# arun-sub/genomicsbench

Hardware: AMD Instinct MI355X
Metric: bsw_large_gcups (higher is better)
Workload: dtype int32

## Files before the change

genomicsbench_amd/csrc/bsw_kernels.hip:

```cpp
#include "gbx_internal.h"
#include <atomic>
#include <climits>
#include <cstdlib>

namespace gbx {
namespace {

constexpr int NEG = -(1 << 29);
constexpr int BIGJ = 1 << 20;

constexpr int NCLS = 21;
constexpr int CLS_LDS = NCLS - 1;
constexpr int NTB = 32;
constexpr int NBIN = NCLS * NTB;
constexpr int HDR = 1024;
constexpr int REG_SCORE_LIMIT = 1 << 20;

struct BswDev {
    int o_del, e_del, o_ins, e_ins, oe_del, oe_ins, zdrop, end_bonus, w, max_mat;
    uint32_t colword[5];
    int32_t col4[5];
    uint32_t row0[5];
    uint32_t row1[5];
    uint8_t remap[24];
    uint32_t lrow[5];
    int lane_on;
};

struct BswPairs {
    const uint8_t *ref, *qer;
    const int64_t *idr, *idq;
    const int32_t *len1, *len2, *h0;
    gbx_bsw_result *out;
    int packed = 0;
};

constexpr int WS_HDR = 4 * HDR;
struct BswWork {
    int32_t *counts, *cursors, *base, *bad, *order, *wband;
    int32_t *lbase, *lrank, *lorder, *lchunk;
};

__host__ __device__ inline int cls_of(int qlen, int bound)
{
    if (qlen > 1024 || bound >= REG_SCORE_LIMIT) return CLS_LDS;
    if (qlen > 256) return 19;
    if (qlen <= 128) return (qlen - 1) >> 3;
    return qlen <= 160 ? 16 : qlen <= 192 ? 17 : 18;
}
constexpr int LANE_QMAX = 159;
constexpr int LANE_ROWS = 2 * (LANE_QMAX + 1);
constexpr int LANE_BINS = LANE_ROWS * 256;
constexpr int LANE_SCORE_LIMIT = 8192;
constexpr int LANE_COMPACT_LIMIT = 256;
constexpr int LANE_NRANGE = 5;
constexpr int LANE_RANGE_HI[2][LANE_NRANGE] = {{47, 79, 99, 135, LANE_QMAX}, {39, 79, 103, 127, LANE_QMAX}};
__host__ __device__ inline bool lane_ok(int lane_on, int qlen, int tlen, int h0, int max_mat)
{
    return lane_on && qlen >= 1 && qlen <= LANE_QMAX && tlen >= 1 && h0 >= 0 && h0 + qlen * (max_mat > 0 ? max_mat : 0) < LANE_SCORE_LIMIT;
}
__host__ __device__ inline int lane_key(int qlen, int h0, int max_mat)
{
    const int wide = h0 + qlen * (max_mat > 0 ? max_mat : 0) < LANE_COMPACT_LIMIT ? 0 : 1;
    return ((wide * (LANE_QMAX + 1) + qlen) << 8) | (h0 < 255 ? h0 : 255);
}

__host__ __device__ inline int bin_of(int cls, int tlen)
{
    const int tb = tlen >> 4;
    return cls * NTB + (NTB - 1 - (tb < NTB - 1 ? tb : NTB - 1));
}

__device__ inline int imax3(int a, int b, int c) { return max(max(a, b), c); }

template <int CTRL, int ROWMASK = 0xf, int BANKMASK = 0xf>
__device__ inline int dpp(int old, int x)
{
    return __builtin_amdgcn_update_dpp(old, x, CTRL, ROWMASK, BANKMASK, false);
}

template <int CTRL, int ROWMASK = 0xf>
__device__ inline int dppz(int x)
{
    return __builtin_amdgcn_mov_dpp(x, CTRL, ROWMASK, 0xf, true);
}

template <int LPP>
__device__ inline int group_scan_max(int x)
{
    if (LPP == 2) return max(x, dppz<0xa0>(x));
    if (LPP <= 8) {
        x = max(x, dppz<0x90>(x));
        x = max(x, dppz<0x40>(x));
        if (LPP == 8) {
            const int tot = dppz<0xff>(x);
            x = max(x, dpp<0x114, 0xf, 0xa>(0, tot));
        }
        return x;
    }
    x = max(x, dppz<0x111>(x));
    x = max(x, dppz<0x112>(x));
    x = max(x, dppz<0x114>(x));
    x = max(x, dppz<0x118>(x));
    if (LPP >= 32) x = max(x, dpp<0x142, 0xa>(NEG, x));
    if (LPP >= 64) x = max(x, dpp<0x143, 0xc>(NEG, x));
    return x;
}

template <int LPP>
__device__ inline int group_shift_up(int x, int fill, int gl)
{
    if (LPP == 16) return dpp<0x111>(fill, x);
    if (LPP < 16) { const int y = dpp<0x111>(fill, x); return gl == 0 ? fill : y; }
    int y = dpp<0x138>(fill, x);
    return gl == 0 ? fill : y;
}

template <int LPP>
__device__ inline int group_allmax(int x)
{
    if (LPP == 2) return max(x, dppz<0xb1>(x));
    if (LPP <= 8) {
        x = max(x, dppz<0xb1>(x));
        x = max(x, dppz<0x4e>(x));
        if (LPP == 8) x = max(x, dppz<0x141>(x));
        return x;
    }
    if (LPP == 16) {
        x = max(x, dppz<0x121>(x));
        x = max(x, dppz<0x122>(x));
        x = max(x, dppz<0x124>(x));
        x = max(x, dppz<0x128>(x));
        return x;
    }
    x = max(x, dpp<0x111>(x, x));
    x = max(x, dpp<0x112>(x, x));
    x = max(x, dpp<0x114>(x, x));
    x = max(x, dpp<0x118>(x, x));
    x = max(x, dpp<0x142, 0xa>(x, x));
    x = max(x, dpp<0x143, 0xc>(x, x));
    return __builtin_amdgcn_readlane(x, 63);
}

__device__ inline int band_width(const BswDev &prm, int qlen)
{
    const int n_ins = qlen * prm.max_mat + prm.end_bonus - prm.o_ins;
    const int n_del = qlen * prm.max_mat + prm.end_bonus - prm.o_del;
    const int l_ins = n_ins >= 0 ? n_ins / prm.e_ins + 1 : 1;
    const int l_del = n_del >= 0 ? n_del / prm.e_del + 1 : 1;
    return min(prm.w, min(l_ins, l_del));
}

constexpr int CLS_THREADS = 1024;
__global__ void __launch_bounds__(CLS_THREADS) bsw_classify_kernel(BswDev prm, BswPairs P, int64_t n, BswWork W, int pass)
{
    __shared__ int lcount[NBIN];
    __shared__ int lbase[NBIN];
    const int tid = threadIdx.x;
    for (int b = tid; b < NBIN; b += CLS_THREADS) lcount[b] = 0;
    __syncthreads();
    const int64_t k = (int64_t)blockIdx.x * CLS_THREADS + tid;
    int bin = -1, slot = 0;
    if (k < n) {
        const int qlen = P.len2[k], tlen = P.len1[k], h0 = P.h0[k];
        if (qlen < 0 || tlen < 0 || qlen > GBX_BSW_MAX_QLEN || tlen > GBX_BSW_MAX_TLEN) {
            if (pass == 0) {
                gbx_bsw_result r = {-1, -1, -1, -1, -1, -1};
                P.out[k] = r;
                atomicAdd(W.bad, 1);
            }
        } else if (tlen == 0 || qlen == 0) {
            if (pass == 0) {
                gbx_bsw_result r;
                r.score = h0; r.tle = 0; r.qle = 0; r.max_off = 0;
                if (tlen == 0) { r.gtle = 0; r.gscore = -1; }
                else { int left = max(h0 - (prm.o_del + prm.e_del), 0); r.gtle = 1; r.gscore = max(-1, left); }
                P.out[k] = r;
            }
        } else if (lane_ok(prm.lane_on, qlen, tlen, h0, prm.max_mat)) {
        } else {
            const int bound = max(h0, 0) + qlen * max(prm.max_mat, 0);
            bin = bin_of(prm.remap[cls_of(qlen, bound)], tlen);
            slot = atomicAdd(&lcount[bin], 1);
        }
    }
    __syncthreads();
    if (pass == 0) {
        for (int b = tid; b < NBIN; b += CLS_THREADS)
            if (lcount[b]) atomicAdd(&W.counts[b], lcount[b]);
        return;
    }
    for (int b = tid; b < NBIN; b += CLS_THREADS)
        lbase[b] = lcount[b] ? W.base[b] + atomicAdd(&W.cursors[b], lcount[b]) : 0;
    __syncthreads();
    if (bin >= 0) {
        W.order[lbase[bin] + slot] = (int)k;
        W.wband[lbase[bin] + slot] = band_width(prm, P.len2[k]);
    }
}

__global__ void __launch_bounds__(HDR) bsw_scan_kernel(BswWork W)
{
    __shared__ int tmp[HDR];
    const int tid = threadIdx.x;
    const int v = tid < NBIN ? W.counts[tid] : 0;
    tmp[tid] = v;
    __syncthreads();
    for (int d = 1; d < HDR; d <<= 1) {
        const int add = tid >= d ? tmp[tid - d] : 0;
        __syncthreads();
        tmp[tid] += add;
        __syncthreads();
    }
    if (tid <= NBIN) W.base[tid] = tmp[tid] - v;
}

constexpr int rows_min_waves(int cpl) { return cpl >= 17 ? 3 : cpl >= 12 ? 4 : cpl >= 9 ? 5 : cpl >= 7 ? 6 : cpl >= 5 ? 7 : 1; }

template <int LPP, int CPL, bool SYM>
__global__ void __launch_bounds__(256, rows_min_waves(CPL)) bsw_rows_kernel(BswDev prm, BswPairs P, BswWork W, int cls)
{
    constexpr int KB = 10;
    constexpr int GROUPS_PER_BLOCK = 256 / LPP;
    constexpr int NQ = (CPL + 3) / 4;
    static_assert(LPP * CPL <= (1 << KB), "column index must fit the key");
    static_assert(CPL <= 32, "in-lane column index uses 5 bits");

    __shared__ uint2 s_row[8];
    const int tid = threadIdx.x;
    if (tid < 8) s_row[tid] = make_uint2(prm.row0[min(tid, 4)], prm.row1[min(tid, 4)]);
    __syncthreads();

    const int gl = tid & (LPP - 1);
    const int j0 = gl * CPL;
    const int ngroups = gridDim.x * GROUPS_PER_BLOCK;
    int next = blockIdx.x * GROUPS_PER_BLOCK + tid / LPP;

    const bool direct = cls < 0;
    const int first = direct ? 0 : W.base[cls * NTB];
    const int cnt = direct ? -cls : W.base[(cls + 1) * NTB] - first;
    const int32_t *order = W.order + first;
    const int32_t *wband = W.wband + first;

    const int e_ins = prm.e_ins, e_del = prm.e_del, oe_ins = prm.oe_ins, oe_del = prm.oe_del;
    const int lane_tilt = gl * (CPL * e_ins);

    int Hs[CPL + 1], Ev[CPL];
    uint32_t Qp[NQ];
#pragma unroll
    for (int c = 0; c < CPL; ++c) { Hs[c] = 0; Ev[c] = 0; }
#pragma unroll
    for (int c = 0; c < NQ; ++c) Qp[c] = 0;

    int qlen = 1, tlen = 1, w = 0, beg = 0, end = 0, i = 0, pair = 0, lq = 0;
    int best = 0, best_i = -1, best_j = -1, g_i = -1, g_score = -1, off = 0;
    int leftv = 0;
    const uint8_t *tptr = P.ref;
    uint2 rcur = s_row[0];
    int tnext = 0;
    bool active = false, done = false;

    for (;;) {
        if (done) {
            if (gl == lq) {
                gbx_bsw_result r;
                r.score = best; r.tle = best_i + 1; r.gtle = g_i + 1; r.qle = best_j + 1;
                r.gscore = g_score; r.max_off = off;
                P.out[pair] = r;
            }
            done = false; active = false;
            tptr = P.ref; tlen = 1; i = 0;
        }
        if (!active && next < cnt) {
            pair = direct ? next : order[next];
            w = direct ? band_width(prm, P.len2[pair]) : wband[next];
            next += ngroups;
            qlen = P.len2[pair]; tlen = P.len1[pair];
            const int h0 = P.h0[pair];
            const uint8_t *q = P.qer + P.idq[pair];
            tptr = P.ref + P.idr[pair];
#pragma unroll
            for (int c = 0; c < NQ; ++c) Qp[c] = 0;
#pragma unroll
            for (int c = 0; c < CPL; ++c) {
                const int j = j0 + c;
                int qc = j < qlen ? q[j] : 0;
                qc = min(qc, 4);
                Qp[c >> 2] |= (uint32_t)qc << ((c & 3) * 8);
                Hs[c] = j == 0 ? h0 : max(h0 - oe_ins - (j - 1) * e_ins, 0);
                Ev[c] = 0;
            }
            lq = (qlen - 1) / CPL;
            leftv = h0 - prm.o_del - e_del;
            best = h0; best_i = -1; best_j = -1; g_i = -1; g_score = -1; off = 0;
            beg = 0; end = qlen; i = 0;
            rcur = s_row[min((int)tptr[0], 4)];
            tnext = tptr[min(1, tlen - 1)];
            active = true;
        }
        if (!__any(active)) break;

        const int b = max(beg, i - w);
        const int e = min(min(end, i + w + 1), qlen);
        const int left0 = b == 0 ? max(leftv, 0) : 0;
        leftv -= e_del;
        const int lo = b - j0, hi = e - j0;
        uint32_t sw[NQ];
#pragma unroll
        for (int k = 0; k < NQ; ++k) sw[k] = __builtin_amdgcn_perm(rcur.y, rcur.x, Qp[k]);
        rcur = s_row[min(tnext, 4)];
        tnext = tptr[min(i + 2, tlen - 1)];

        int G[CPL];
        int lf = NEG;
#pragma unroll
        for (int c = 0; c < CPL; ++c) {
            const bool p = (c >= lo) & (c < hi);
            const int hsv = Hs[c];
            const int sc = (int)(int8_t)(sw[c >> 2] >> ((c & 3) * 8));
            const int m = (p & (hsv != 0)) ? hsv + sc : 0;
            const int ein = p ? Ev[c] : 0;
            G[c] = imax3(m, ein, lf);
            const int mo = m - oe_ins;
            lf = imax3(lf - e_ins, mo, 0);
            Ev[c] = imax3(ein - e_del, SYM ? mo : m - oe_del, 0);
        }
        const int carry = group_scan_max<LPP>(lf + lane_tilt) - lane_tilt;
        int X = group_shift_up<LPP>(carry, NEG, gl);

        int kl = 0, hl = 0;
#pragma unroll
        for (int c = 0; c < CPL; ++c) {
            int h = max(G[c], X);
            X -= e_ins;
            const bool pr = c < hi;
            Hs[c + 1] = pr ? h : Hs[c + 1];
            hl = pr ? h : hl;
            h = pr ? h : 0;
            G[c] = h;
            kl = max(kl, (h << 5) | c);
        }
        const int hin = group_shift_up<LPP>(G[CPL - 1], left0, gl);
        Hs[0] = hi >= 0 ? hin : Hs[0];
        unsigned zm = 0;
#pragma unroll
        for (int c = 0; c < CPL; ++c) {
            const int hs = c == 0 ? hin : G[c - 1];
            unsigned nz;
            asm("v_min_u32_e32 %0, 1, %1" : "=v"(nz) : "v"(hs | Ev[c]));
            zm |= nz << c;
        }
        Hs[CPL] = 0;

        const int key = group_allmax<LPP>(((kl >> 5) << KB) | (j0 + (kl & 31)));
        const int m = key >> KB, mj = key & ((1 << KB) - 1);
        const int zf_l = zm ? j0 + (__builtin_ffs((int)zm) - 1) : BIGJ;
        const int zl_l = zm ? j0 + (31 - __builtin_clz(zm)) : -1;
        const int zfirst = BIGJ - group_allmax<LPP>(BIGJ - zf_l);
        const int zlast = group_allmax<LPP>(zl_l);

        const bool live = b < e;
        const int jfin = live ? e : b;
        const int hend = live ? hl : left0;
        const bool gq = jfin == qlen;
        g_i = (gq & (hend >= g_score)) ? i : g_i;
        g_score = gq ? max(g_score, hend) : g_score;
        const bool upd = (m > best) & (m != 0);
        const int dd = (i - best_i) - (mj - best_j);
        const int pen = max(__mul24(dd, e_del), __mul24(-dd, e_ins));
        const bool zbrk = (prm.zdrop > 0) & !upd & (best - m - pen > prm.zdrop);
        const bool brk = (m == 0) | zbrk;
        const int dmi = mj - i;
        off = upd ? imax3(off, dmi, -dmi) : off;
        best_i = upd ? i : best_i;
        best_j = upd ? mj : best_j;
        best = upd ? m : best;
        beg = min(zfirst, e);
        end = min(zlast + 2, qlen);
        ++i;
        done = active & (brk | (i >= tlen));
    }
}

__global__ void __launch_bounds__(64) bsw_lds_kernel(BswDev prm, BswPairs P, BswWork W, int cls)
{
    extern __shared__ int lds[];
    const int lane = threadIdx.x;
    const int first = W.base[cls * NTB];
    const int cnt = W.base[(cls + 1) * NTB] - first;
    const int32_t *order = W.order + first;
    const int e_ins = prm.e_ins, e_del = prm.e_del, oe_ins = prm.oe_ins, oe_del = prm.oe_del;

    for (int slot = blockIdx.x; slot < cnt; slot += gridDim.x) {
        const int pair = order[slot];
        const int qlen = P.len2[pair], tlen = P.len1[pair], h0 = P.h0[pair];
        const uint8_t *q = P.qer + P.idq[pair];
        const uint8_t *tp = P.ref + P.idr[pair];
        int *hd = lds, *ev = lds + (qlen + 1);
        for (int j = lane; j <= qlen; j += 64) {
            hd[j] = j == 0 ? h0 : max(h0 - oe_ins - (j - 1) * e_ins, 0);
            ev[j] = 0;
        }
        __syncthreads();
        int w;
        {
            int lim = (int)((double)(qlen * prm.max_mat + prm.end_bonus - prm.o_ins) / (double)e_ins + 1.);
            lim = max(lim, 1); w = min(prm.w, lim);
            lim = (int)((double)(qlen * prm.max_mat + prm.end_bonus - prm.o_del) / (double)e_del + 1.);
            lim = max(lim, 1); w = min(w, lim);
        }
        int best = h0, best_i = -1, best_j = -1, g_i = -1, g_score = -1, off = 0;
        int beg = 0, end = qlen;
        for (int i = 0; i < tlen; ++i) {
            const int b = max(beg, i - w);
            const int e = min(min(end, i + w + 1), qlen);
            const int left0 = b == 0 ? max(h0 - (prm.o_del + e_del * (i + 1)), 0) : 0;
            const int t = min((int)tp[i], 4);
            int fcarry = NEG;
            int left = left0;
            int m = 0, mj = -1;
            int zfirst = BIGJ, zlast = -1;
            if (left0 != 0) { zfirst = b; zlast = b; }
            for (int cb = b; cb < e; cb += 64) {
                const int j = cb + lane;
                const bool p = j < e;
                const int qc = p ? min((int)q[j], 4) : 0;
                const int s = t == 4 ? prm.col4[qc] : (int)(int8_t)(prm.colword[qc] >> (t << 3));
                const int hsv = p ? hd[j] : 0;
                const int ein = p ? ev[j] : 0;
                const int mm = (p & (hsv != 0)) ? hsv + s : 0;
                const int src = p ? max(mm - oe_ins, 0) : NEG;
                int pre = group_scan_max<64>(src + lane * e_ins);
                int fincl = pre - lane * e_ins;
                int fexcl = group_shift_up<64>(fincl, NEG, lane);
                fexcl = lane == 0 ? NEG : fexcl - 0;
                const int f = max(fexcl, fcarry - lane * e_ins);
                int h = imax3(mm, ein, f);
                h = p ? h : 0;
                const int enew = imax3(ein - e_del, mm - oe_del, 0);
                {
                    const int tot = __builtin_amdgcn_readlane(fincl, 63);
                    fcarry = max(tot, fcarry - 64 * e_ins);
                }
                int hprev = group_shift_up<64>(h, left, lane);
                hprev = lane == 0 ? left : hprev;
                left = __builtin_amdgcn_readlane(h, 63);
                if (p) { hd[j] = hprev; ev[j] = enew; }
                {
                    const int hm = group_allmax<64>(h);
                    if (hm >= m && (hm > 0 || m == 0)) {
                        const unsigned long long eq = __ballot(p && h == hm);
                        if (eq) { mj = cb + 63 - __builtin_clzll(eq); m = hm; }
                    }
                    const unsigned long long nzh = __ballot(p && h != 0);
                    const unsigned long long nze = __ballot(p && enew != 0);
                    if (nzh) {
                        zfirst = min(zfirst, cb + (int)__builtin_ctzll(nzh) + 1);
                        zlast = max(zlast, cb + 63 - (int)__builtin_clzll(nzh) + 1);
                    }
                    if (nze) {
                        zfirst = min(zfirst, cb + (int)__builtin_ctzll(nze));
                        zlast = max(zlast, cb + 63 - (int)__builtin_clzll(nze));
                    }
                }
                if (cb + 64 >= e) left = __builtin_amdgcn_readlane(h, (e - 1 - cb) & 63);
            }
            if (lane == 0) { hd[e] = b < e ? left : left0; ev[e] = 0; }
            __syncthreads();
            const int hend = b < e ? left : left0;
            const int jfin = b < e ? e : b;
            if (jfin == qlen) { g_i = g_score > hend ? g_i : i; g_score = max(g_score, hend); }
            if (m == 0) break;
            if (m > best) {
                best = m; best_i = i; best_j = mj; off = max(off, abs(mj - i));
            } else if (prm.zdrop > 0) {
                const int di = i - best_i, dj = mj - best_j;
                const int pen = di > dj ? (di - dj) * e_del : (dj - di) * e_ins;
                if (best - m - pen > prm.zdrop) break;
            }
            beg = min(zfirst, e);
            end = min(zlast + 2, qlen);
        }
        if (lane == 0) {
            gbx_bsw_result r;
            r.score = best; r.tle = best_i + 1; r.gtle = g_i + 1; r.qle = best_j + 1;
            r.gscore = g_score; r.max_off = off;
            P.out[pair] = r;
        }
        __syncthreads();
    }
}

__global__ void __launch_bounds__(256) bsw_lane_sort_kernel(BswDev prm, BswPairs P, int64_t n, BswWork W, int pass)
{
    const int64_t k = (int64_t)blockIdx.x * 256 + threadIdx.x;
    if (k >= n) return;
    const int qlen = P.len2[k], tlen = P.len1[k], h0 = P.h0[k];
    if (!lane_ok(prm.lane_on, qlen, tlen, h0, prm.max_mat) || tlen > GBX_BSW_MAX_TLEN) return;
    const int key = lane_key(qlen, h0, prm.max_mat);
    if (pass == 0) W.lrank[k] = atomicAdd(&W.lbase[key + 1], 1);
    else W.lorder[W.lbase[key] + W.lrank[k]] = (int)k;
}
__global__ void __launch_bounds__(1024) bsw_lane_scan_kernel(BswWork W)
{
    constexpr int PER = (LANE_BINS + 1023) / 1024;
    __shared__ int part[1024];
    const int tid = threadIdx.x;
    int sum = 0;
    for (int k = 0; k < PER; ++k) { const int b = tid * PER + k; if (b < LANE_BINS) sum += W.lbase[b + 1]; }
    part[tid] = sum;
    __syncthreads();
    for (int d = 1; d < 1024; d <<= 1) {
        const int add = tid >= d ? part[tid - d] : 0;
        __syncthreads();
        part[tid] += add;
        __syncthreads();
    }
    int run = part[tid] - sum;
    for (int k = 0; k < PER; ++k) {
        const int b = tid * PER + k;
        if (b < LANE_BINS) { const int c = W.lbase[b + 1]; run += c; W.lbase[b + 1] = run; }
    }
}

template <bool SYM>
__device__ __forceinline__ uint32_t lane_pair_step(uint32_t w, uint32_t qq, uint32_t rw, uint32_t rwn, int &f, int &left, uint32_t kin, uint32_t &key, int pa, int pa1,
                                                   int zero, int oe_del, int oe_ins, int e_del, int e_ins)
{
    uint32_t wn, kout;
    int hb;
    if (SYM) {
        int sa, ta, tb, ma, mb, x, ha, td, ed, ena, enb, fd, ka, kb, u, v;
        asm volatile(
            "v_perm_b32 %[sa], %[rwn], %[rw], %[qq]\n"
            "v_cmp_ne_u32_sdwa vcc, %[w], %[zero] src0_sel:BYTE_1 src1_sel:DWORD\n"
            "v_subrev_u32 %[fd], %[eins], %[f]\n"
            "v_add_u32_sdwa %[ta], sext(%[sa]), %[w] dst_sel:DWORD dst_unused:UNUSED_PAD src0_sel:BYTE_0 src1_sel:BYTE_1\n"
            "v_cndmask_b32 %[ma], 0, %[ta], vcc\n"
            "v_cmp_ne_u32_sdwa vcc, %[w], %[zero] src0_sel:BYTE_3 src1_sel:DWORD\n"
            "v_max_i32_sdwa %[x], %[ma], %[w] dst_sel:DWORD dst_unused:UNUSED_PAD src0_sel:DWORD src1_sel:BYTE_0\n"
            "v_add_u32_sdwa %[tb], sext(%[sa]), %[w] dst_sel:DWORD dst_unused:UNUSED_PAD src0_sel:BYTE_1 src1_sel:BYTE_3\n"
            "v_max_i32 %[ha], %[x], %[f]\n"
            "v_subrev_u32 %[td], %[oed], %[ma]\n"
            "v_cndmask_b32 %[mb], 0, %[tb], vcc\n"
            "v_sub_u32_sdwa %[ed], %[w], %[edel] dst_sel:DWORD dst_unused:UNUSED_PAD src0_sel:BYTE_0 src1_sel:DWORD\n"
            "v_max3_i32 %[f], %[fd], %[td], 0\n"
            "v_max3_i32 %[ena], %[ed], %[td], 0\n"
            "v_max_i32_sdwa %[x], %[mb], %[w] dst_sel:DWORD dst_unused:UNUSED_PAD src0_sel:DWORD src1_sel:BYTE_2\n"
            "v_lshl_or_b32 %[ka], %[ha], 18, %[pa]\n"
            "v_max_i32 %[hb], %[x], %[f]\n"
            "v_subrev_u32 %[td], %[oed], %[mb]\n"
            "v_subrev_u32 %[fd], %[eins], %[f]\n"
            "v_sub_u32_sdwa %[ed], %[w], %[edel] dst_sel:DWORD dst_unused:UNUSED_PAD src0_sel:BYTE_2 src1_sel:DWORD\n"
            "v_max3_i32 %[f], %[fd], %[td], 0\n"
            "v_max3_i32 %[enb], %[ed], %[td], 0\n"
            "v_lshl_or_b32 %[kb], %[hb], 18, %[pa1]\n"
            "v_lshl_or_b32 %[u], %[left], 8, %[ena]\n"
            "v_lshl_or_b32 %[v], %[ha], 8, %[enb]\n"
            "v_max3_u32 %[key], %[kin], %[ka], %[kb]\n"
            "v_lshl_or_b32 %[wn], %[v], 16, %[u]\n"
            : [sa] "=&v"(sa), [ta] "=&v"(ta), [tb] "=&v"(tb), [ma] "=&v"(ma), [mb] "=&v"(mb), [x] "=&v"(x), [ha] "=&v"(ha),
              [hb] "=&v"(hb), [td] "=&v"(td), [ed] "=&v"(ed), [ena] "=&v"(ena), [enb] "=&v"(enb), [fd] "=&v"(fd), [ka] "=&v"(ka),
              [kb] "=&v"(kb), [u] "=&v"(u), [v] "=&v"(v), [wn] "=&v"(wn), [f] "+v"(f), [key] "=v"(kout)
            : [w] "v"(w), [qq] "v"(qq), [rw] "v"(rw), [rwn] "v"(rwn), [left] "v"(left), [kin] "v"(kin), [pa] "v"(pa), [pa1] "v"(pa1), [zero] "v"(zero), [oed] "s"(oe_del),
              [edel] "s"(e_del), [eins] "s"(e_ins)
            : "vcc");
    } else {
        int sa, ta, tb, ma, mb, x, ha, td, ti, ed, ena, enb, fd, ka, kb, u, v;
        asm volatile(
            "v_perm_b32 %[sa], %[rwn], %[rw], %[qq]\n"
            "v_cmp_ne_u32_sdwa vcc, %[w], %[zero] src0_sel:BYTE_1 src1_sel:DWORD\n"
            "v_subrev_u32 %[fd], %[eins], %[f]\n"
            "v_add_u32_sdwa %[ta], sext(%[sa]), %[w] dst_sel:DWORD dst_unused:UNUSED_PAD src0_sel:BYTE_0 src1_sel:BYTE_1\n"
            "v_cndmask_b32 %[ma], 0, %[ta], vcc\n"
            "v_cmp_ne_u32_sdwa vcc, %[w], %[zero] src0_sel:BYTE_3 src1_sel:DWORD\n"
            "v_max_i32_sdwa %[x], %[ma], %[w] dst_sel:DWORD dst_unused:UNUSED_PAD src0_sel:DWORD src1_sel:BYTE_0\n"
            "v_add_u32_sdwa %[tb], sext(%[sa]), %[w] dst_sel:DWORD dst_unused:UNUSED_PAD src0_sel:BYTE_1 src1_sel:BYTE_3\n"
            "v_max_i32 %[ha], %[x], %[f]\n"
            "v_subrev_u32 %[td], %[oed], %[ma]\n"
            "v_subrev_u32 %[ti], %[oei], %[ma]\n"
            "v_cndmask_b32 %[mb], 0, %[tb], vcc\n"
            "v_sub_u32_sdwa %[ed], %[w], %[edel] dst_sel:DWORD dst_unused:UNUSED_PAD src0_sel:BYTE_0 src1_sel:DWORD\n"
            "v_max3_i32 %[f], %[fd], %[ti], 0\n"
            "v_max3_i32 %[ena], %[ed], %[td], 0\n"
            "v_max_i32_sdwa %[x], %[mb], %[w] dst_sel:DWORD dst_unused:UNUSED_PAD src0_sel:DWORD src1_sel:BYTE_2\n"
            "v_lshl_or_b32 %[ka], %[ha], 18, %[pa]\n"
            "v_max_i32 %[hb], %[x], %[f]\n"
            "v_subrev_u32 %[td], %[oed], %[mb]\n"
            "v_subrev_u32 %[ti], %[oei], %[mb]\n"
            "v_subrev_u32 %[fd], %[eins], %[f]\n"
            "v_sub_u32_sdwa %[ed], %[w], %[edel] dst_sel:DWORD dst_unused:UNUSED_PAD src0_sel:BYTE_2 src1_sel:DWORD\n"
            "v_max3_i32 %[f], %[fd], %[ti], 0\n"
            "v_max3_i32 %[enb], %[ed], %[td], 0\n"
            "v_lshl_or_b32 %[kb], %[hb], 18, %[pa1]\n"
            "v_lshl_or_b32 %[u], %[left], 8, %[ena]\n"
            "v_lshl_or_b32 %[v], %[ha], 8, %[enb]\n"
            "v_max3_u32 %[key], %[kin], %[ka], %[kb]\n"
            "v_lshl_or_b32 %[wn], %[v], 16, %[u]\n"
            : [sa] "=&v"(sa), [ta] "=&v"(ta), [tb] "=&v"(tb), [ma] "=&v"(ma), [mb] "=&v"(mb), [x] "=&v"(x), [ha] "=&v"(ha),
              [hb] "=&v"(hb), [td] "=&v"(td), [ti] "=&v"(ti), [ed] "=&v"(ed), [ena] "=&v"(ena), [enb] "=&v"(enb), [fd] "=&v"(fd), [ka] "=&v"(ka),
              [kb] "=&v"(kb), [u] "=&v"(u), [v] "=&v"(v), [wn] "=&v"(wn), [f] "+v"(f), [key] "=v"(kout)
            : [w] "v"(w), [qq] "v"(qq), [rw] "v"(rw), [rwn] "v"(rwn), [left] "v"(left), [kin] "v"(kin), [pa] "v"(pa), [pa1] "v"(pa1), [zero] "v"(zero), [oed] "s"(oe_del),
              [oei] "s"(oe_ins), [edel] "s"(e_del), [eins] "s"(e_ins)
            : "vcc");
    }
    left = hb;
    key = kout;
    return wn;
}

#ifdef GBX_BSW_LANE_STATS
__device__ unsigned long long g_bsw_lane_stats[16][4];
#endif
template <bool SYM, bool COMPACT, bool CODE4 = false, bool PACKED = false>
__global__ void __launch_bounds__(64) bsw_lane_kernel(BswDev prm, BswPairs P, BswWork W, int rlo, int rhi, int cols, int slot)
{
    extern __shared__ uint32_t lcell[];
#ifdef GBX_BSW_LANE_STATS
    __shared__ int st_rowmax[2048];
    for (int k = threadIdx.x; k < 2048; k += 64) st_rowmax[k] = 0;
    unsigned long long st_cells = 0, st_rows = 0, st_wcells = 0, st_wrows = 0;
#endif
#define LCELL(byte_addr) (*(uint32_t *)((char *)lcell + (byte_addr)))
#define LCELL16(byte_addr) (*(uint16_t *)((char *)lcell + (byte_addr)))
#define LQ8(byte_addr) (*((uint8_t *)lcell + (byte_addr)))
    const int lane = threadIdx.x;
    const int first = W.lbase[rlo << 8], count = W.lbase[(rhi + 1) << 8] - first;
    const int nchunks = (count + 63) >> 6;
    const int32_t *order = W.lorder + first;
    const int e_ins = prm.e_ins, e_del = prm.e_del, oe_ins = prm.oe_ins, oe_del = prm.oe_del;
    const int cb = lane * 4;
    constexpr int QROW = CODE4 ? 64 : 128;
    const int qb = (cols >> 1) * 256 + (CODE4 ? lane : (lane & 31) * 4 + (lane >> 5) * 2);
    auto LQREAD = [&](int a) -> uint32_t { return CODE4 ? (uint32_t)LQ8(a) : (uint32_t)LCELL16(a); };
    auto QSEL = [](uint32_t q) -> uint32_t { return CODE4 ? (((q >> 4) << 8) | (q & 15u)) : q; };
    auto QLOW = [](uint32_t q) -> uint32_t { return CODE4 ? (q & 15u) : (q & 0xffu); };
    auto cell_at = [&](int j) { return COMPACT ? (j >> 1) * 256 + cb + (j & 1) * 2 : j * 256 + cb; };
    const int tab = COMPACT ? (cols >> 1) * (256 + QROW) + 512 : (cols + 2) * 256 - 128;
    if (lane < 5) *(uint4 *)((char *)lcell + tab + lane * 16) = make_uint4(prm.row0[lane], prm.row1[lane], prm.lrow[lane], 0u);
#define LTAB(base_code) (*(const uint4 *)((const char *)lcell + tab + min((int)(base_code), 4) * 16))
    int rel0 = 0, rel1 = 2, rel2 = 256, rel3 = 258, rel4 = 512, rel5 = 514, rel6 = 768, rel7 = 770;
    asm volatile("" : "+v"(rel0), "+v"(rel1), "+v"(rel2), "+v"(rel3), "+v"(rel4), "+v"(rel5), "+v"(rel6), "+v"(rel7));
    for (;;) {
        int c = 0;
        if (lane == 0) c = atomicAdd(&W.lchunk[slot], 1);
        c = __builtin_amdgcn_readfirstlane(c);
        if (c >= nchunks) break;
        const int hi_ = count - (c << 6), idx = hi_ - 64 + lane;
        const bool have = idx >= 0;
        const int pair = order[have ? idx : 0];
        const int qlen = P.len2[pair], tlen = P.len1[pair], h0 = P.h0[pair];
        const int64_t qo = P.idq[pair], to = P.idr[pair];
        const uint8_t *q = P.qer + (PACKED ? 0 : qo);
        const uint8_t *t = P.ref + (PACKED ? 0 : to);
        auto qpiece = [&](int j) -> uint4 {
            uint4 r;
            if (!PACKED) { __builtin_memcpy(&r, q + j, 16); return r; }
            const int64_t o = qo + j;
            const uint8_t *b = q + (o >> 1);
            uint64_t v;
            __builtin_memcpy(&v, b, 8);
            if (o & 1) v = (v >> 4) | ((uint64_t)b[8] << 60);
            auto spread = [](unsigned h) -> unsigned { return (h & 0xfu) | ((h & 0xf0u) << 4) | ((h & 0xf00u) << 8) | ((h & 0xf000u) << 12); };
            const unsigned lo = (unsigned)v, hi = (unsigned)(v >> 32);
            r.x = spread(lo & 0xffffu); r.y = spread(lo >> 16); r.z = spread(hi & 0xffffu); r.w = spread(hi >> 16);
            return r;
        };
        auto tbase = [&](int i) -> int {
            if (!PACKED) return t[i];
            const int64_t o = to + i;
            return (t[o >> 1] >> ((int)(o & 1) * 4)) & 15;
        };
        {
            uint4 wq = qpiece(0);
// ... 586 lines not shown
        d->row1[t] = (uint32_t)(uint8_t)p->mat[t * 5 + 4];
    }
    d->lane_on = 0;
    bool fits6 = true;
    for (int k = 0; k < 25; ++k) fits6 = fits6 && p->mat[k] >= -32 && p->mat[k] <= 31;
    for (int t = 0; t < 5; ++t) {
        uint32_t wv = 0;
        for (int q = 0; q < 5; ++q) wv |= ((uint32_t)p->mat[t * 5 + q] & 63u) << (6 * q);
        d->lrow[t] = wv;
    }
    if (fits6 && p->o_del + p->e_del < LANE_SCORE_LIMIT && p->o_ins + p->e_ins < LANE_SCORE_LIMIT) d->lane_on = -1;
    return GBX_OK;
}

}

constexpr int64_t WS_LANE = (int64_t)(LANE_BINS + 64) + 64;
size_t bsw_workspace_bytes(int64_t n)
{
    return (size_t)(WS_HDR + 4 * (n > 0 ? n : 0) + WS_LANE) * sizeof(int32_t);
}

constexpr int UNPACK_ROUNDS = 4;
__device__ inline unsigned spread4(unsigned h) { return (h & 0xfu) | ((h & 0xf0u) << 4) | ((h & 0xf00u) << 8) | ((h & 0xf000u) << 12); }
__global__ void __launch_bounds__(256) bsw_unpack4_kernel(const uint8_t *__restrict__ packed, uint8_t *__restrict__ out, int64_t lo, int64_t hi)
{
    const int64_t base = lo + (int64_t)blockIdx.x * (256 * 16 * UNPACK_ROUNDS) + threadIdx.x * 16;
    const bool aligned = (((uintptr_t)(packed + (base >> 1)) & 7) == 0) && (((uintptr_t)(out + base) & 15) == 0);
    if (aligned && base + (int64_t)(UNPACK_ROUNDS - 1) * 4096 + 16 <= hi) {
        uint2 v[UNPACK_ROUNDS];
#pragma unroll
        for (int r = 0; r < UNPACK_ROUNDS; ++r) v[r] = *(const uint2 *)(packed + ((base + r * 4096) >> 1));
#pragma unroll
        for (int r = 0; r < UNPACK_ROUNDS; ++r) {
            uint4 q;
            q.x = spread4(v[r].x & 0xffffu); q.y = spread4(v[r].x >> 16); q.z = spread4(v[r].y & 0xffffu); q.w = spread4(v[r].y >> 16);
            *(uint4 *)(out + base + r * 4096) = q;
        }
        return;
    }
    for (int r = 0; r < UNPACK_ROUNDS; ++r) {
        const int64_t o = base + r * 4096;
        if (o >= hi) return;
        if (aligned && o + 16 <= hi) {
            const uint2 v = *(const uint2 *)(packed + (o >> 1));
            uint4 q;
            q.x = spread4(v.x & 0xffffu); q.y = spread4(v.x >> 16); q.z = spread4(v.y & 0xffffu); q.w = spread4(v.y >> 16);
            *(uint4 *)(out + o) = q;
        } else {
            for (int64_t k = o; k < o + 16 && k < hi; ++k) out[k] = (uint8_t)((packed[k >> 1] >> ((k & 1) * 4)) & 0xf);
        }
    }
}

int bsw_unpack4(const uint8_t *d_packed, uint8_t *d_out, int64_t lo, int64_t hi, hipStream_t s)
{
    if (hi <= lo) return GBX_OK;
    const int64_t per_block = 256 * 16 * UNPACK_ROUNDS;
    Stage st("bsw_unpack4", s);
    hipLaunchKernelGGL(bsw_unpack4_kernel, dim3((unsigned)((hi - lo + per_block - 1) / per_block)), dim3(256), 0, s, d_packed, d_out, lo, hi);
    GBX_HIP(hipGetLastError());
    return GBX_OK;
}

int bsw_launch_direct(const gbx_bsw_params *p, int64_t n, int max_qlen,
                      const uint8_t *d_ref, const uint8_t *d_qer, const int64_t *d_idr, const int64_t *d_idq,
                      const int32_t *d_len1, const int32_t *d_len2, const int32_t *d_h0, gbx_bsw_result *d_out, hipStream_t s)
{
    if (n <= 0) return GBX_OK;
    BswDev dev;
    int rc = make_dev_params(p, &dev);
    if (rc) return rc;
    for (int c = 0; c < NCLS; ++c) dev.remap[c] = (uint8_t)c;
    BswPairs P = {d_ref, d_qer, d_idr, d_idq, d_len1, d_len2, d_h0, d_out};
    BswWork W = {nullptr, nullptr, nullptr, nullptr, nullptr, nullptr, nullptr, nullptr, nullptr, nullptr};
    dev.lane_on = 0;
    if (max_qlen > 256) { set_error("bsw: direct launch needs queries of at most 256"); return GBX_ERR_ARG; }
    const int cols = max_qlen + 1;
    int lpp = 16, cpl = cols <= 128 ? 8 : cols <= 160 ? 10 : cols <= 192 ? 12 : 16;
    if (n < 4096) { lpp = 64; cpl = cols <= 192 ? 3 : 4; }
    if (const char *e = getenv("GBX_BSW_DIRECT_SHAPE")) {
        int l = 0, c = 0;
        if (sscanf(e, "%dx%d", &l, &c) == 2 && l * c > max_qlen && find_row_kernel(l, c)) { lpp = l; cpl = c; }
    }
    RowKernel *k = find_row_kernel(lpp, cpl);
    if (!k) { set_error("bsw: no %dx%d row kernel", lpp, cpl); return GBX_ERR_UNSUPPORTED; }
    const bool sym = dev.oe_ins == dev.oe_del;
    const int gpb = 256 / lpp;
    const int blocks = (int)((n + gpb - 1) / gpb);
    Stage st(k->name, s);
    hipLaunchKernelGGL(k->fn[sym], dim3(blocks), dim3(256), 0, s, dev, P, W, -(int)n);
    GBX_HIP(hipGetLastError());
    return GBX_OK;
}

static std::atomic<long long> g_lane_reg_launches{0};

static bool lane_wanted(int64_t n)
{
    const char *lane_env = getenv("GBX_BSW_LANE");
    const int64_t lane_min = getenv("GBX_BSW_LANE_MIN") ? atoll(getenv("GBX_BSW_LANE_MIN")) : 262144;
    return lane_env ? atoi(lane_env) != 0 : n >= lane_min;
}

int bsw_lane_rule(const gbx_bsw_params *p, int64_t n, BswLaneRule *r)
{
    BswDev dev;
    const int rc = make_dev_params(p, &dev);
    if (rc) return rc;
    r->on = dev.lane_on && lane_wanted(n) ? 1 : 0;
    r->max_mat = dev.max_mat > 0 ? dev.max_mat : 0;
    r->qmax = LANE_QMAX;
    r->limit = LANE_SCORE_LIMIT;
    return GBX_OK;
}

struct BswCall {
    BswDev dev; BswPairs P; BswWork W;
    int64_t n;
    int mode, cus;
    bool sym;
    hipStream_t s; SideStreams *ss; hipEvent_t *join_events; const BswChunkPrep *prep;
    bool ahead;
    bool no_rows;
    bool packed_lanes;
    int phase;
    hipStream_t s_cls;
    hipEvent_t ev_pre, ev_aux;
};

static int plan_call(BswCall &c)
{
    const BswChunkPrep *prep = c.prep;
    static const bool prep_off = switched_off("GBX_BSW_PREP");
    c.ahead = prep && prep->uploaded && c.join_events && !prep_off;
    c.s_cls = c.ahead ? c.ss->pre[0] : c.s;
    c.no_rows = c.dev.lane_on && prep && prep->rows_pairs == 0 && !switched_off("GBX_BSW_SKIP_ROWS");
    c.packed_lanes = c.no_rows && prep->ref_packed && !switched_off("GBX_BSW_PACKED_LANES");
    c.phase = prep ? prep->phase : 0;
    if (c.phase && !(c.ahead && c.packed_lanes && prep->ev_pre && prep->ev_aux)) {
        if (c.phase == 1) return 1;
        set_error("bsw: the kernels of a chunk whose preparing passes were not queued");
        return GBX_ERR_ARG;
    }
    c.ev_pre = c.phase ? prep->ev_pre : c.ss->ev_pre;
    c.ev_aux = c.phase ? prep->ev_aux : c.ss->ev_aux;
    if (c.packed_lanes) { c.P.ref = prep->ref_packed; c.P.qer = prep->qer_packed; c.P.packed = 1; }
    return GBX_OK;
}

static int queue_prepare(BswCall &c)
{
    const BswChunkPrep *prep = c.prep;
    SideStreams *ss = c.ss;
    const int64_t n = c.n;
    int rc;
    if (c.ahead) {
        GBX_HIP(hipStreamWaitEvent(ss->pre[0], prep->uploaded, 0));
        GBX_HIP(hipStreamWaitEvent(ss->pre[1], prep->uploaded, 0));
    }
    if (!c.packed_lanes && prep && prep->ref_packed) {
        const int64_t from_r = prep->unp_r ? *prep->unp_r : prep->lo_r, from_q = prep->unp_q ? *prep->unp_q : prep->lo_q;
        if ((rc = bsw_unpack4(prep->ref_packed, prep->ref_bytes, from_r, prep->hi_r, c.s_cls)) ||
            (rc = bsw_unpack4(prep->qer_packed, prep->qer_bytes, from_q, prep->hi_q, c.s_cls)))
            return rc;
        if (prep->unp_r && prep->hi_r > *prep->unp_r) *prep->unp_r = prep->hi_r;
        if (prep->unp_q && prep->hi_q > *prep->unp_q) *prep->unp_q = prep->hi_q;
    }
    GBX_HIP(hipMemsetAsync(c.W.counts, 0, WS_HDR * sizeof(int32_t), c.s_cls));
    if (c.dev.lane_on) {
        hipStream_t so;
        if (c.ahead) {
            so = ss->pre[1];
            GBX_HIP(hipMemsetAsync(c.W.lbase, 0, (size_t)WS_LANE * sizeof(int32_t), so));
        } else {
            GBX_HIP(hipMemsetAsync(c.W.lbase, 0, (size_t)WS_LANE * sizeof(int32_t), c.s));
            if ((rc = ss->fork(c.s))) return rc;
            so = ss->side[SideStreams::N - 1];
        }
        Stage st("bsw_lane_sort", so);
        const int sblocks = (int)((n + 255) / 256);
        hipLaunchKernelGGL(bsw_lane_sort_kernel, dim3(sblocks), dim3(256), 0, so, c.dev, c.P, n, c.W, 0);
        hipLaunchKernelGGL(bsw_lane_scan_kernel, dim3(1), dim3(1024), 0, so, c.W);
        hipLaunchKernelGGL(bsw_lane_sort_kernel, dim3(sblocks), dim3(256), 0, so, c.dev, c.P, n, c.W, 1);
        GBX_HIP(hipEventRecord(c.ev_aux, so));
    }
    const int cblocks = (int)((n + CLS_THREADS - 1) / CLS_THREADS);
    {
        Stage st("bsw_classify", c.s_cls);
        hipLaunchKernelGGL(bsw_classify_kernel, dim3(cblocks), dim3(CLS_THREADS), 0, c.s_cls, c.dev, c.P, n, c.W, 0);
        hipLaunchKernelGGL(bsw_scan_kernel, dim3(1), dim3(HDR), 0, c.s_cls, c.W);
        hipLaunchKernelGGL(bsw_classify_kernel, dim3(cblocks), dim3(CLS_THREADS), 0, c.s_cls, c.dev, c.P, n, c.W, 1);
    }
    if (c.ahead) GBX_HIP(hipEventRecord(c.ev_pre, c.s_cls));
    GBX_HIP(hipGetLastError());
    return GBX_OK;
}

static int kernel_streams_wait(const BswCall &c, hipEvent_t ev, int n_side = SideStreams::N)
{
    GBX_HIP(hipStreamWaitEvent(c.s, ev, 0));
    for (int k = 0; k < n_side; ++k) GBX_HIP(hipStreamWaitEvent(c.ss->side[k], ev, 0));
    return GBX_OK;
}

static void launch_row_classes(BswCall &c)
{
    const int nk = c.join_events ? 3 : 4;
    int launched = 0;
    for (int cls = 0; cls < NCLS - 1; ++cls) {
        if (CLASS_REMAP[c.mode][cls] != cls) continue;
        const int sk = (c.mode ? launched++ : cls) % nk;
        hipStream_t sc = c.dev.lane_on || sk == 0 ? c.s : c.ss->side[sk - 1];
        RowKernel &k = row_kernels[cls];
        const int bpc = resident_blocks(k.bpc[c.sym], (const void *)k.fn[c.sym], 256, 2, 8);
        const int gpb = 256 / k.lpp;
        const int64_t want = (c.n + gpb - 1) / gpb, cap = (int64_t)c.cus * bpc;
        Stage st(k.name, sc);
        hipLaunchKernelGGL(k.fn[c.sym], dim3((int)(want < cap ? want : cap)), dim3(256), 0, sc, c.dev, c.P, c.W, cls);
    }
}

static void launch_lane_reg(const BswCall &c, hipStream_t sc, int64_t want, int rlo, int rhi, int slot)
{
    static_assert(LANE_RANGE_HI[0][2] == 99, "bsw_lane_reg_kernel instance");
    typedef void (*LaneRegFn)(BswDev, BswPairs, BswWork, int, int, int);
    static const LaneRegFn reg_fn[2] = {bsw_lane_reg_kernel<false, 99>, bsw_lane_reg_kernel<true, 99>};
    static std::atomic<int> reg_bpc[2];
    const int64_t cap = (int64_t)c.cus * resident_blocks(reg_bpc[c.sym], (const void *)reg_fn[c.sym], 64, 8, INT_MAX);
    hipLaunchKernelGGL(reg_fn[c.sym], dim3((unsigned)(want < cap ? want : cap)), dim3(64), 0, sc, c.dev, c.P, c.W, rlo, rhi, slot);
    g_lane_reg_launches.fetch_add(1, std::memory_order_relaxed);
}

static void launch_lanes(const BswCall &c)
{
    static const char *names[2][LANE_NRANGE] = {{"bsw_lane_c47", "bsw_lane_c79", "bsw_lane_c99", "bsw_lane_c135", "bsw_lane_c159"},
                                                {"bsw_lane_w39", "bsw_lane_w79", "bsw_lane_w103", "bsw_lane_w127", "bsw_lane_w159"}};
    const int64_t want = (c.n + 63) / 64;
    for (int fmt = 1; fmt >= 0; --fmt) {
        for (int r = LANE_NRANGE - 1; r >= 0; --r) {
            const int qlo = r ? LANE_RANGE_HI[fmt][r - 1] + 1 : 1, qhi = LANE_RANGE_HI[fmt][r];
            const int cols = (qhi + 3) & ~1;
            const int kind = fmt ? LANE_WIDE : qhi > 99 ? LANE_COMPACT4 : LANE_COMPACT;
            const size_t lds = fmt ? (size_t)(cols + 2) * 256 : (size_t)(cols / 2) * (kind == LANE_COMPACT4 ? 320 : 384) + 640;
            const int fit = (int)((size_t)160 * 1024 / lds), per_cu = fit > 16 ? 16 : fit;
            const int sk = (LANE_NRANGE - 1 - r) & 3;
            hipStream_t sc = sk == 0 ? c.s : c.ss->side[sk - 1];
            const int64_t cap = (int64_t)c.cus * per_cu;
            const int rlo = fmt * (LANE_QMAX + 1) + qlo, rhi = fmt * (LANE_QMAX + 1) + qhi, slot = fmt * LANE_NRANGE + r;
            Stage st(names[fmt][r], sc);
            if (fmt == 0 && !c.P.packed && qhi == 99 && !switched_off("GBX_BSW_LANE_REG")) { launch_lane_reg(c, sc, want, rlo, rhi, slot); continue; }
            hipLaunchKernelGGL(lane_kernels[c.P.packed][kind][c.sym], dim3((unsigned)(want < cap ? want : cap)), dim3(64), lds, sc,
                               c.dev, c.P, c.W, rlo, rhi, cols, slot);
        }
    }
}

static int launch_lds(const BswCall &c)
{
    const size_t lds_bytes = (size_t)(GBX_BSW_MAX_QLEN + 1) * 2 * sizeof(int);
    static std::atomic<uint64_t> attr_set[2];
    int cur = 0;
    GBX_HIP(hipGetDevice(&cur));
    const uint64_t bit = (uint64_t)1 << (cur & 63);
    if (cur >= 128 || !(attr_set[cur >> 6].load(std::memory_order_acquire) & bit)) {
        GBX_HIP(hipFuncSetAttribute((const void *)bsw_lds_kernel, hipFuncAttributeMaxDynamicSharedMemorySize, (int)lds_bytes));
        if (cur < 128) attr_set[cur >> 6].fetch_or(bit, std::memory_order_release);
    }
    const int blocks = (int)(c.n < (int64_t)c.cus * 2 ? c.n : (int64_t)c.cus * 2);
    Stage st("bsw_lds", c.s);
    hipLaunchKernelGGL(bsw_lds_kernel, dim3(blocks), dim3(64), lds_bytes, c.s, c.dev, c.P, c.W, CLS_LDS);
    return GBX_OK;
}

int bsw_launch(const gbx_bsw_params *p, int64_t n,
               const uint8_t *d_ref, const uint8_t *d_qer,
               const int64_t *d_idr, const int64_t *d_idq,
               const int32_t *d_len1, const int32_t *d_len2, const int32_t *d_h0,
               gbx_bsw_result *d_out, void *d_work, size_t work_bytes, hipStream_t s, hipEvent_t *join_events,
               const BswChunkPrep *prep)
{
    if (n == 0) return GBX_OK;
    if (n > 0x7fffffffLL - 1024) { set_error("bsw: more than 2^31 pairs in one call"); return GBX_ERR_UNSUPPORTED; }
    if (work_bytes < bsw_workspace_bytes(n)) { set_error("bsw: workspace too small"); return GBX_ERR_ARG; }
    BswCall c;
    int rc = make_dev_params(p, &c.dev);
    if (rc) return rc;
    c.n = n; c.mode = class_mode_for(n); c.cus = 256;
    for (int k = 0; k < NCLS; ++k) c.dev.remap[k] = CLASS_REMAP[c.mode][k];
    c.P = {d_ref, d_qer, d_idr, d_idq, d_len1, d_len2, d_h0, d_out};
    int32_t *wi = (int32_t *)d_work, *wl = wi + WS_HDR + 4 * n;
    c.W = {wi, wi + HDR, wi + 2 * HDR, wi + 3 * HDR, wi + WS_HDR, wi + WS_HDR + n, wl, wi + WS_HDR + 3 * n, wi + WS_HDR + 2 * n, wl + LANE_BINS + 64};
    c.dev.lane_on = c.dev.lane_on && lane_wanted(n) ? 1 : 0;
    c.sym = c.dev.oe_ins == c.dev.oe_del;
    c.s = s; c.join_events = join_events; c.prep = prep;
    if ((rc = side_streams(&c.ss))) return rc;
    std::unique_lock<std::mutex> side_lock(c.ss->mu);
    if ((rc = plan_call(c))) return rc;
    if (c.phase != 2) {
        if ((rc = queue_prepare(c))) return rc;
        if (c.phase == 1) return GBX_OK;
    }
    if (c.ahead) {
        if ((rc = kernel_streams_wait(c, c.ev_pre))) return rc;
        if (c.phase == 2 && (rc = kernel_streams_wait(c, prep->uploaded))) return rc;
    }
    int dev_id = 0;
    (void)hipGetDevice(&dev_id);
    (void)hipDeviceGetAttribute(&c.cus, hipDeviceAttributeMultiprocessorCount, dev_id);
    if (!c.dev.lane_on && !c.ahead && (rc = c.ss->fork(s))) return rc;
    if (!c.no_rows) launch_row_classes(c);
    if (c.dev.lane_on) {
        if ((rc = kernel_streams_wait(c, c.ev_aux, c.ahead ? SideStreams::N : SideStreams::N - 1))) return rc;
        launch_lanes(c);
    }
    if (!join_events && (rc = c.ss->join(s))) return rc;
    if (!c.no_rows && (rc = launch_lds(c))) return rc;
    if (join_events) {
        GBX_HIP(hipEventRecord(join_events[0], s));
        for (int k = 0; k < SideStreams::N; ++k) GBX_HIP(hipEventRecord(join_events[1 + k], c.ss->side[k]));
    }
    GBX_HIP(hipGetLastError());
    return GBX_OK;
}

}

extern "C" long long gbx_debug_bsw_lane_reg_launches(void)
{
    return gbx::g_lane_reg_launches.load(std::memory_order_relaxed);
}

#ifdef GBX_BSW_LANE_STATS
extern "C" int gbx_debug_bsw_lane_stats(unsigned long long *out, int reset)
{
    if (hipMemcpyFromSymbol(out, HIP_SYMBOL(gbx::g_bsw_lane_stats), sizeof(unsigned long long) * 64) != hipSuccess) return -1;
    if (reset) { unsigned long long z[64] = {0}; if (hipMemcpyToSymbol(HIP_SYMBOL(gbx::g_bsw_lane_stats), z, sizeof(z)) != hipSuccess) return -1; }
    return 0;
}
#endif
```

Measured before the change: 2525.

## Fold lane sort into classify passes and scan both histograms in one kernel

```diff
diff --git a/genomicsbench_amd/csrc/bsw_kernels.hip b/genomicsbench_amd/csrc/bsw_kernels.hip
--- a/genomicsbench_amd/csrc/bsw_kernels.hip
+++ b/genomicsbench_amd/csrc/bsw_kernels.hip
@@ -160,9 +160,10 @@
     for (int b = tid; b < NBIN; b += CLS_THREADS) lcount[b] = 0;
     __syncthreads();
     const int64_t k = (int64_t)blockIdx.x * CLS_THREADS + tid;
-    int bin = -1, slot = 0;
+    int bin = -1, slot = 0, key = -1, qlen = 0;
     if (k < n) {
-        const int qlen = P.len2[k], tlen = P.len1[k], h0 = P.h0[k];
+        qlen = P.len2[k];
+        const int tlen = P.len1[k], h0 = P.h0[k];
         if (qlen < 0 || tlen < 0 || qlen > GBX_BSW_MAX_QLEN || tlen > GBX_BSW_MAX_TLEN) {
             if (pass == 0) {
                 gbx_bsw_result r = {-1, -1, -1, -1, -1, -1};
@@ -178,41 +179,75 @@
                 P.out[k] = r;
             }
         } else if (lane_ok(prm.lane_on, qlen, tlen, h0, prm.max_mat)) {
+            key = lane_key(qlen, h0, prm.max_mat);
         } else {
             const int bound = max(h0, 0) + qlen * max(prm.max_mat, 0);
             bin = bin_of(prm.remap[cls_of(qlen, bound)], tlen);
             slot = atomicAdd(&lcount[bin], 1);
         }
     }
-    __syncthreads();
     if (pass == 0) {
+        if (key >= 0) W.lrank[k] = atomicAdd(&W.lbase[key], 1);
+        __syncthreads();
         for (int b = tid; b < NBIN; b += CLS_THREADS)
             if (lcount[b]) atomicAdd(&W.counts[b], lcount[b]);
         return;
     }
+    __syncthreads();
     for (int b = tid; b < NBIN; b += CLS_THREADS)
         lbase[b] = lcount[b] ? W.base[b] + atomicAdd(&W.cursors[b], lcount[b]) : 0;
     __syncthreads();
+    if (key >= 0) W.lorder[W.lbase[key] + W.lrank[k]] = (int)k;
     if (bin >= 0) {
         W.order[lbase[bin] + slot] = (int)k;
-        W.wband[lbase[bin] + slot] = band_width(prm, P.len2[k]);
-    }
-}
-
-__global__ void __launch_bounds__(HDR) bsw_scan_kernel(BswWork W)
-{
-    __shared__ int tmp[HDR];
-    const int tid = threadIdx.x;
+        W.wband[lbase[bin] + slot] = band_width(prm, qlen);
+    }
+}
+
+__device__ inline int wave_scan_add(int x)
+{
+    x += dppz<0x111>(x);
+    x += dppz<0x112>(x);
+    x += dppz<0x114>(x);
+    x += dppz<0x118>(x);
+    x += dpp<0x142, 0xa>(0, x);
+    x += dpp<0x143, 0xc>(0, x);
+    return x;
+}
+
+constexpr int SCAN_ROWS = LANE_BINS / (16 * 64);
+static_assert(SCAN_ROWS * 16 * 64 == LANE_BINS && HDR == 1024 && NBIN < HDR, "bsw_scan_kernel's tiling");
+__global__ void __launch_bounds__(HDR) bsw_scan_kernel(BswWork W, int lane_on)
+{
+    __shared__ int wtot[2][16];
+    const int tid = threadIdx.x, lane = tid & 63, wave = tid >> 6;
     const int v = tid < NBIN ? W.counts[tid] : 0;
-    tmp[tid] = v;
+    int32_t *lb = W.lbase + wave * (SCAN_ROWS * 64) + lane;
+    int c[SCAN_ROWS], carry = 0;
+    if (lane_on) {
+#pragma unroll
+        for (int r = 0; r < SCAN_ROWS; ++r) c[r] = lb[r * 64];
+    }
+    const int incl = wave_scan_add(v);
+    if (lane == 63) wtot[0][wave] = incl;
+    if (lane_on) {
+#pragma unroll
+        for (int r = 0; r < SCAN_ROWS; ++r) {
+            const int in = wave_scan_add(c[r]);
+            c[r] = carry + in - c[r];
+            carry += __builtin_amdgcn_readlane(in, 63);
+        }
+    }
+    if (lane == 0) wtot[1][wave] = carry;
     __syncthreads();
-    for (int d = 1; d < HDR; d <<= 1) {
-        const int add = tid >= d ? tmp[tid - d] : 0;
-        __syncthreads();
-        tmp[tid] += add;
-        __syncthreads();
-    }
-    if (tid <= NBIN) W.base[tid] = tmp[tid] - v;
+    int before = 0, lbefore = 0;
+    for (int w = 0; w < wave; ++w) { before += wtot[0][w]; lbefore += wtot[1][w]; }
+    if (tid <= NBIN) W.base[tid] = before + incl - v;
+    if (lane_on) {
+#pragma unroll
+        for (int r = 0; r < SCAN_ROWS; ++r) lb[r * 64] = lbefore + c[r];
+        if (tid == HDR - 1) W.lbase[LANE_BINS] = lbefore + carry;
+    }
 }
 
 constexpr int rows_min_waves(int cpl) { return cpl >= 17 ? 3 : cpl >= 12 ? 4 : cpl >= 9 ? 5 : cpl >= 7 ? 6 : cpl >= 5 ? 7 : 1; }
@@ -488,38 +523,6 @@
             P.out[pair] = r;
         }
         __syncthreads();
-    }
-}
-
-__global__ void __launch_bounds__(256) bsw_lane_sort_kernel(BswDev prm, BswPairs P, int64_t n, BswWork W, int pass)
-{
-    const int64_t k = (int64_t)blockIdx.x * 256 + threadIdx.x;
-    if (k >= n) return;
-    const int qlen = P.len2[k], tlen = P.len1[k], h0 = P.h0[k];
-    if (!lane_ok(prm.lane_on, qlen, tlen, h0, prm.max_mat) || tlen > GBX_BSW_MAX_TLEN) return;
-    const int key = lane_key(qlen, h0, prm.max_mat);
-    if (pass == 0) W.lrank[k] = atomicAdd(&W.lbase[key + 1], 1);
-    else W.lorder[W.lbase[key] + W.lrank[k]] = (int)k;
-}
-__global__ void __launch_bounds__(1024) bsw_lane_scan_kernel(BswWork W)
-{
-    constexpr int PER = (LANE_BINS + 1023) / 1024;
-    __shared__ int part[1024];
-    const int tid = threadIdx.x;
-    int sum = 0;
-    for (int k = 0; k < PER; ++k) { const int b = tid * PER + k; if (b < LANE_BINS) sum += W.lbase[b + 1]; }
-    part[tid] = sum;
-    __syncthreads();
-    for (int d = 1; d < 1024; d <<= 1) {
-        const int add = tid >= d ? part[tid - d] : 0;
-        __syncthreads();
-        part[tid] += add;
-        __syncthreads();
-    }
-    int run = part[tid] - sum;
-    for (int k = 0; k < PER; ++k) {
-        const int b = tid * PER + k;
-        if (b < LANE_BINS) { const int c = W.lbase[b + 1]; run += c; W.lbase[b + 1] = run; }
     }
 }
 
@@ -1412,13 +1415,9 @@
 static int queue_prepare(BswCall &c)
 {
     const BswChunkPrep *prep = c.prep;
-    SideStreams *ss = c.ss;
     const int64_t n = c.n;
     int rc;
-    if (c.ahead) {
-        GBX_HIP(hipStreamWaitEvent(ss->pre[0], prep->uploaded, 0));
-        GBX_HIP(hipStreamWaitEvent(ss->pre[1], prep->uploaded, 0));
-    }
+    if (c.ahead) GBX_HIP(hipStreamWaitEvent(c.s_cls, prep->uploaded, 0));
     if (!c.packed_lanes && prep && prep->ref_packed) {
         const int64_t from_r = prep->unp_r ? *prep->unp_r : prep->lo_r, from_q = prep->unp_q ? *prep->unp_q : prep->lo_q;
         if ((rc = bsw_unpack4(prep->ref_packed, prep->ref_bytes, from_r, prep->hi_r, c.s_cls)) ||
@@ -1427,40 +1426,26 @@
         if (prep->unp_r && prep->hi_r > *prep->unp_r) *prep->unp_r = prep->hi_r;
         if (prep->unp_q && prep->hi_q > *prep->unp_q) *prep->unp_q = prep->hi_q;
     }
-    GBX_HIP(hipMemsetAsync(c.W.counts, 0, WS_HDR * sizeof(int32_t), c.s_cls));
-    if (c.dev.lane_on) {
-        hipStream_t so;
-        if (c.ahead) {
-            so = ss->pre[1];
-            GBX_HIP(hipMemsetAsync(c.W.lbase, 0, (size_t)WS_LANE * sizeof(int32_t), so));
-        } else {
-            GBX_HIP(hipMemsetAsync(c.W.lbase, 0, (size_t)WS_LANE * sizeof(int32_t), c.s));
-            if ((rc = ss->fork(c.s))) return rc;
-            so = ss->side[SideStreams::N - 1];
-        }
-        Stage st("bsw_lane_sort", so);
-        const int sblocks = (int)((n + 255) / 256);
-        hipLaunchKernelGGL(bsw_lane_sort_kernel, dim3(sblocks), dim3(256), 0, so, c.dev, c.P, n, c.W, 0);
-        hipLaunchKernelGGL(bsw_lane_scan_kernel, dim3(1), dim3(1024), 0, so, c.W);
-        hipLaunchKernelGGL(bsw_lane_sort_kernel, dim3(sblocks), dim3(256), 0, so, c.dev, c.P, n, c.W, 1);
-        GBX_HIP(hipEventRecord(c.ev_aux, so));
-    }
+    GBX_HIP(hipMemsetAsync(c.W.counts, 0, (size_t)(WS_HDR + (c.dev.lane_on ? WS_LANE : 0)) * sizeof(int32_t), c.s_cls));
     const int cblocks = (int)((n + CLS_THREADS - 1) / CLS_THREADS);
     {
         Stage st("bsw_classify", c.s_cls);
         hipLaunchKernelGGL(bsw_classify_kernel, dim3(cblocks), dim3(CLS_THREADS), 0, c.s_cls, c.dev, c.P, n, c.W, 0);
-        hipLaunchKernelGGL(bsw_scan_kernel, dim3(1), dim3(HDR), 0, c.s_cls, c.W);
+        hipLaunchKernelGGL(bsw_scan_kernel, dim3(1), dim3(HDR), 0, c.s_cls, c.W, c.dev.lane_on);
         hipLaunchKernelGGL(bsw_classify_kernel, dim3(cblocks), dim3(CLS_THREADS), 0, c.s_cls, c.dev, c.P, n, c.W, 1);
     }
-    if (c.ahead) GBX_HIP(hipEventRecord(c.ev_pre, c.s_cls));
+    if (c.ahead) {
+        GBX_HIP(hipEventRecord(c.ev_pre, c.s_cls));
+        GBX_HIP(hipEventRecord(c.ev_aux, c.s_cls));
+    }
     GBX_HIP(hipGetLastError());
     return GBX_OK;
 }
 
-static int kernel_streams_wait(const BswCall &c, hipEvent_t ev, int n_side = SideStreams::N)
+static int kernel_streams_wait(const BswCall &c, hipEvent_t ev)
 {
     GBX_HIP(hipStreamWaitEvent(c.s, ev, 0));
-    for (int k = 0; k < n_side; ++k) GBX_HIP(hipStreamWaitEvent(c.ss->side[k], ev, 0));
+    for (int k = 0; k < SideStreams::N; ++k) GBX_HIP(hipStreamWaitEvent(c.ss->side[k], ev, 0));
     return GBX_OK;
 }
 
@@ -1549,8 +1534,8 @@
     c.n = n; c.mode = class_mode_for(n); c.cus = 256;
     for (int k = 0; k < NCLS; ++k) c.dev.remap[k] = CLASS_REMAP[c.mode][k];
     c.P = {d_ref, d_qer, d_idr, d_idq, d_len1, d_len2, d_h0, d_out};
-    int32_t *wi = (int32_t *)d_work, *wl = wi + WS_HDR + 4 * n;
-    c.W = {wi, wi + HDR, wi + 2 * HDR, wi + 3 * HDR, wi + WS_HDR, wi + WS_HDR + n, wl, wi + WS_HDR + 3 * n, wi + WS_HDR + 2 * n, wl + LANE_BINS + 64};
+    int32_t *wi = (int32_t *)d_work, *wl = wi + WS_HDR, *wn = wl + WS_LANE;
+    c.W = {wi, wi + HDR, wi + 2 * HDR, wi + 3 * HDR, wn, wn + n, wl, wn + 3 * n, wn + 2 * n, wl + LANE_BINS + 64};
     c.dev.lane_on = c.dev.lane_on && lane_wanted(n) ? 1 : 0;
     c.sym = c.dev.oe_ins == c.dev.oe_del;
     c.s = s; c.join_events = join_events; c.prep = prep;
@@ -1564,18 +1549,16 @@
     if (c.ahead) {
         if ((rc = kernel_streams_wait(c, c.ev_pre))) return rc;
         if (c.phase == 2 && (rc = kernel_streams_wait(c, prep->uploaded))) return rc;
-    }
+    } else if ((rc = c.ss->fork(s))) return rc;
     int dev_id = 0;
     (void)hipGetDevice(&dev_id);
     (void)hipDeviceGetAttribute(&c.cus, hipDeviceAttributeMultiprocessorCount, dev_id);
-    if (!c.dev.lane_on && !c.ahead && (rc = c.ss->fork(s))) return rc;
-    if (!c.no_rows) launch_row_classes(c);
-    if (c.dev.lane_on) {
-        if ((rc = kernel_streams_wait(c, c.ev_aux, c.ahead ? SideStreams::N : SideStreams::N - 1))) return rc;
-        launch_lanes(c);
-    }
+    if (!c.no_rows) {
+        launch_row_classes(c);
+        if ((rc = launch_lds(c))) return rc;
+    }
+    if (c.dev.lane_on) launch_lanes(c);
     if (!join_events && (rc = c.ss->join(s))) return rc;
-    if (!c.no_rows && (rc = launch_lds(c))) return rc;
     if (join_events) {
         GBX_HIP(hipEventRecord(join_events[0], s));
         for (int k = 0; k < SideStreams::N; ++k) GBX_HIP(hipEventRecord(join_events[1 + k], c.ss->side[k]));
```

Result: no change. 2539 (median of 2 runs) (+0.6%).
